# SciLifeLab/TIDDIT

Measured on AMD Instinct MI355X. Metric: cov bins/sec, 30x WGS synthetic (signals clustered/sec: see 'dbscan'), higher is better.
Workload: dtype int64; 1 GPU; BASELINE configs[1]: coverage histogram, 24 contigs x 125000000 bp (3.00 Gb), 30x 150-bp sorted stream, 500-bp bins, q>=20 filter; contigs split over the 1 rank(s); reads=600000000, bins=6000000

## Files before the change

tiddit_amd/csrc/tdt_coverage.hip:

```cpp
extern const char *const tdt_variant_coverage;
const char *const tdt_variant_coverage = ""
#ifdef COV_MIN_WAVES
    " COV_MIN_WAVES"
#endif
#ifdef COV_MIN_WAVES1
    " COV_MIN_WAVES1"
#endif
#ifdef COV_MIN_WAVES1_4
    " COV_MIN_WAVES1_4"
#endif
#ifdef COV_MIN_WAVES4
    " COV_MIN_WAVES4"
#endif
#ifdef COV_RPL
    " COV_RPL"
#endif
#ifdef COV_RPL1
    " COV_RPL1"
#endif
#ifdef COV_SPARES1
    " COV_SPARES1"
#endif
#ifdef COV_WIN
    " COV_WIN"
#endif
#ifdef COV_WIN1
    " COV_WIN1"
#endif
    ;

#include "tdt_common.h"

#include <algorithm>
#include <thread>

#define COV_THREADS 256
#ifndef COV_RPL
#define COV_RPL 8
#endif
#ifndef COV_RPL1
#define COV_RPL1 4
#endif
#define COV_READS_PER_BLOCK 16384
#ifndef COV_WIN
#define COV_WIN 2048
#endif
#define COV_LUT_LDS_MAX 1024
#define COV_PUSH_CHUNK (4u << 20)
#define COV_STATUS_BYTES (128 + COV_KEPT_SLOTS * 128)
#define COV_KEPT_SLOTS 512

struct CovItem {
    const int32_t *start;
    const int32_t *end;
    const uint8_t *mapq;
    const uint16_t *flag;
    const unsigned long long *packed;
    unsigned long long n;
    unsigned long long *acc;
    const unsigned long long *lut_end;
    int nbins;
    int aligned;
    unsigned first_block;
    unsigned binned;
};

struct CovParams {
    CovItem it;
    const CovItem *items;
    int n_items;
    int bin_size;
    unsigned magic;
    int shift;
    int min_q;
    int margin;
    unsigned xmax, m15;
    int k15;
    const unsigned long long *lut_main;
    unsigned long long one;
    int *status;
    unsigned long long *kept;
};

__device__ __forceinline__ int cov_div(int x, unsigned magic, int shift) {
    return shift < 0 ? x : (int)(__umulhi((unsigned)x, magic) >> shift);
}

#define DPP_WAVE_SHL1 0x130
#define DPP_WAVE_SHR1 0x138

template <int CTRL>
__device__ __forceinline__ unsigned long long dpp_u64(unsigned long long v) {
    const unsigned lo = __builtin_amdgcn_update_dpp(0u, (unsigned)v, CTRL, 0xf, 0xf, true);
    const unsigned hi = __builtin_amdgcn_update_dpp(0u, (unsigned)(v >> 32), CTRL, 0xf, 0xf, true);
    return ((unsigned long long)hi << 32) | lo;
}

#define COV_DPP_SHR1 "row_shr:1 row_mask:0xf bank_mask:0xf bound_ctrl:0"
#define COV_DPP_SHR2 "row_shr:2 row_mask:0xf bank_mask:0xf bound_ctrl:0"
#define COV_DPP_SHR4 "row_shr:4 row_mask:0xf bank_mask:0xf bound_ctrl:0"
#define COV_DPP_SHR8 "row_shr:8 row_mask:0xf bank_mask:0xf bound_ctrl:0"
#define COV_DPP_BC15 "row_bcast:15 row_mask:0xa bank_mask:0xf"
#define COV_DPP_BC31 "row_bcast:31 row_mask:0xc bank_mask:0xf"
#define COV_SCAN_ALL(STEP) \
    "s_nop 1\n\t" STEP(COV_DPP_SHR1) STEP(COV_DPP_SHR2) STEP(COV_DPP_SHR4) STEP(COV_DPP_SHR8) STEP(COV_DPP_BC15) STEP(COV_DPP_BC31) "s_nop 1"
#define COV_SCAN_STEP(CTRL)                                                                     \
    "v_add_co_u32_dpp %0, vcc, %0, %0 " CTRL "\n\t"                                             \
    "v_addc_co_u32_dpp %1, vcc, %1, %1, vcc " CTRL "\n\t"                                       \
    "v_add_co_u32_dpp %2, vcc, %2, %2 " CTRL "\n\t"                                             \
    "v_addc_co_u32_dpp %3, vcc, %3, %3, vcc " CTRL "\n\t"                                       \
    "v_add_co_u32_dpp %4, vcc, %4, %4 " CTRL "\n\t"                                             \
    "v_addc_co_u32_dpp %5, vcc, %5, %5, vcc " CTRL "\n\t"

__device__ __forceinline__ void wave_scan3_u64(unsigned long long &a0, unsigned long long &a1, unsigned long long &a2) {
    unsigned l0 = (unsigned)a0, h0 = (unsigned)(a0 >> 32), l1 = (unsigned)a1, h1 = (unsigned)(a1 >> 32),
             l2 = (unsigned)a2, h2 = (unsigned)(a2 >> 32);
    asm volatile(COV_SCAN_ALL(COV_SCAN_STEP) : "+v"(l0), "+v"(h0), "+v"(l1), "+v"(h1), "+v"(l2), "+v"(h2)::"vcc", "memory");
    a0 = ((unsigned long long)h0 << 32) | l0;
    a1 = ((unsigned long long)h1 << 32) | l1;
    a2 = ((unsigned long long)h2 << 32) | l2;
}

__device__ __forceinline__ unsigned long long cov_mask_lt(unsigned a, unsigned lim_uniform) {
    unsigned long long m;
    asm("v_cmp_gt_u32_e64 %0, %1, %2" : "=s"(m) : "s"(lim_uniform), "v"(a));
    return m;
}
__device__ __forceinline__ unsigned long long cov_mask_eq0(unsigned a) {
    unsigned long long m;
    asm("v_cmp_eq_u32_e64 %0, 0, %1" : "=s"(m) : "v"(a));
    return m;
}
__device__ __forceinline__ unsigned long long cov_mask_ne0(unsigned a) {
    unsigned long long m;
    asm("v_cmp_ne_u32_e64 %0, 0, %1" : "=s"(m) : "v"(a));
    return m;
}
__device__ __forceinline__ unsigned cov_select(unsigned long long m, unsigned if_set, unsigned if_clear) {
    unsigned r;
    asm("v_cndmask_b32_e64 %0, %1, %2, %3" : "=v"(r) : "v"(if_clear), "v"(if_set), "s"(m));
    return r;
}

#define COV_SCAN2_STEP(CTRL)                                                                    \
    "v_add_co_u32_dpp %0, vcc, %0, %0 " CTRL "\n\t"                                             \
    "v_addc_co_u32_dpp %1, vcc, %1, %1, vcc " CTRL "\n\t"                                       \
    "v_add_co_u32_dpp %2, vcc, %2, %2 " CTRL "\n\t"                                             \
    "v_addc_co_u32_dpp %3, vcc, %3, %3, vcc " CTRL "\n\t"

__device__ __forceinline__ void wave_scan2_u64(unsigned long long &a0, unsigned long long &a1) {
    unsigned l0 = (unsigned)a0, h0 = (unsigned)(a0 >> 32), l1 = (unsigned)a1, h1 = (unsigned)(a1 >> 32);
    asm volatile(COV_SCAN_ALL(COV_SCAN2_STEP) : "+v"(l0), "+v"(h0), "+v"(l1), "+v"(h1)::"vcc", "memory");
    a0 = ((unsigned long long)h0 << 32) | l0;
    a1 = ((unsigned long long)h1 << 32) | l1;
}

#define COV_SCAN4I_STEP(CTRL)                                                                   \
    "v_add_u32_dpp %0, %0, %0 " CTRL "\n\t"                                                     \
    "v_add_u32_dpp %1, %1, %1 " CTRL "\n\t"                                                     \
    "v_add_u32_dpp %2, %2, %2 " CTRL "\n\t"                                                     \
    "v_add_u32_dpp %3, %3, %3 " CTRL "\n\t"

__device__ __forceinline__ void wave_scan4_i32(int &p0, int &p1, int &p2, int &p3) {
    asm volatile(COV_SCAN_ALL(COV_SCAN4I_STEP) : "+v"(p0), "+v"(p1), "+v"(p2), "+v"(p3)::"memory");
}

__device__ __forceinline__ ulonglong2 cov_lds_read128(unsigned addr) {
#if defined(__HIP_DEVICE_COMPILE__)
    typedef unsigned long long cov_v2u64 __attribute__((ext_vector_type(2)));
    const cov_v2u64 v = *reinterpret_cast<const cov_v2u64 __attribute__((address_space(3))) *>(addr);
    return make_ulonglong2(v.x, v.y);
#else
    (void)addr;
    return make_ulonglong2(0, 0);
#endif
}

__device__ __forceinline__ unsigned long long cov_lds_read64(unsigned addr) {
#if defined(__HIP_DEVICE_COMPILE__)
    return *reinterpret_cast<const unsigned long long __attribute__((address_space(3))) *>(addr);
#else
    return addr;
#endif
}
__device__ __forceinline__ void cov_lds_add64(unsigned addr, unsigned long long v) {
#if defined(__HIP_DEVICE_COMPILE__)
    __hip_atomic_fetch_add(reinterpret_cast<unsigned long long __attribute__((address_space(3))) *>(addr), v, __ATOMIC_RELAXED, __HIP_MEMORY_SCOPE_WORKGROUP);
#else
    (void)addr; (void)v;
#endif
}
__device__ __forceinline__ unsigned cov_add_bit(unsigned r, unsigned long long mask) {
    unsigned out;
    unsigned long long cout;
    asm("v_addc_co_u32_e64 %0, %1, %2, 0, %3" : "=v"(out), "=s"(cout) : "v"(r), "s"(mask));
    return out;
}

__device__ __noinline__ void cov_global_add(unsigned long long *acc, int bin, unsigned long long v) {
    atomicAdd(&acc[bin], v);
}

template <int RPL>
struct CovTile {
    int s[RPL], e[RPL];
    unsigned mq[RPL / 4];
    unsigned fl[RPL / 2];
};

template <int RPL>
__device__ __forceinline__ CovTile<RPL> cov_load(const CovItem &P, unsigned long long idx, unsigned long long r1) {
    CovTile<RPL> t;
    if (P.aligned && idx + RPL <= r1) {
#pragma unroll
        for (int k = 0; k < RPL / 4; k++) {
            const int4 s4 = *reinterpret_cast<const int4 *>(P.start + idx + 4 * k);
            const int4 e4 = *reinterpret_cast<const int4 *>(P.end + idx + 4 * k);
            t.s[4 * k] = s4.x; t.s[4 * k + 1] = s4.y; t.s[4 * k + 2] = s4.z; t.s[4 * k + 3] = s4.w;
            t.e[4 * k] = e4.x; t.e[4 * k + 1] = e4.y; t.e[4 * k + 2] = e4.z; t.e[4 * k + 3] = e4.w;
        }
        if (RPL == 8) {
            const uint2 m2 = *reinterpret_cast<const uint2 *>(P.mapq + idx);
            const uint4 f4 = *reinterpret_cast<const uint4 *>(P.flag + idx);
            t.mq[0] = m2.x; t.mq[RPL / 4 - 1] = m2.y;
            t.fl[0] = f4.x; t.fl[1] = f4.y; t.fl[RPL / 2 - 2] = f4.z; t.fl[RPL / 2 - 1] = f4.w;
        } else {
            t.mq[0] = *reinterpret_cast<const unsigned *>(P.mapq + idx);
            const uint2 f2 = *reinterpret_cast<const uint2 *>(P.flag + idx);
            t.fl[0] = f2.x; t.fl[1] = f2.y;
        }
    } else {
#pragma unroll
        for (int k = 0; k < RPL / 4; k++) t.mq[k] = 0;
#pragma unroll
        for (int k = 0; k < RPL / 2; k++) t.fl[k] = 0;
#pragma unroll
        for (int j = 0; j < RPL; j++) {
            const bool ok = idx + j < r1;
            t.s[j] = ok ? P.start[idx + j] : 0;
            t.e[j] = ok ? P.end[idx + j] : 1;
            t.mq[j / 4] |= (ok ? (unsigned)P.mapq[idx + j] : 0u) << (8 * (j & 3));
            t.fl[j / 2] |= (ok ? (unsigned)P.flag[idx + j] : 0x4u) << (16 * (j & 1));
        }
    }
    return t;
}

template <int RPL>
struct CovTileP {
    unsigned long long w[RPL];
};

template <int RPL>
__device__ __forceinline__ CovTileP<RPL> cov_load_packed(const CovItem &P, unsigned long long idx, unsigned long long r1) {
    CovTileP<RPL> t;
    if (P.aligned && idx + RPL <= r1) {
#pragma unroll
        for (int k = 0; k < RPL / 2; k++) {
            const ulonglong2 v = *reinterpret_cast<const ulonglong2 *>(P.packed + idx + 2 * k);
            t.w[2 * k] = v.x;
            t.w[2 * k + 1] = v.y;
        }
    } else {
#pragma unroll
        for (int j = 0; j < RPL; j++) t.w[j] = idx + j < r1 ? P.packed[idx + j] : (1ull << 62);
    }
    return t;
}

__global__ void cov_pack(const int32_t *__restrict__ start, const int32_t *__restrict__ end, const uint8_t *__restrict__ mapq,
                         const uint16_t *__restrict__ flag, unsigned long long n, unsigned long long *__restrict__ out) {
    unsigned long long i = (unsigned long long)blockIdx.x * blockDim.x + threadIdx.x;
    const unsigned long long stride = (unsigned long long)gridDim.x * blockDim.x;
    for (; i < n; i += stride) out[i] = cov_pack_record(start[i], end[i], mapq[i], flag[i]);
}

__global__ void cov_pack_binned(const int32_t *__restrict__ start, const int32_t *__restrict__ end, const uint8_t *__restrict__ mapq,
                                const uint16_t *__restrict__ flag, unsigned long long n, int nbins, unsigned z, unsigned magic, int shift, int mode1,
                                unsigned long long *__restrict__ out) {
    unsigned long long i = (unsigned long long)blockIdx.x * blockDim.x + threadIdx.x;
    const unsigned long long stride = (unsigned long long)gridDim.x * blockDim.x;
    for (; i < n; i += stride) out[i] = cov_bin_record(start[i], end[i], mapq[i], flag[i], nbins, z, magic, shift, mode1 != 0);
}

#define COV_DBIT 48
#define COV_LOWMASK ((1ull << COV_DBIT) - 1ull)
#ifndef COV_WIN1
#define COV_WIN1 2048
#endif
#define COV_DQMAX 256
#ifndef COV_SPARES1
#define COV_SPARES1 64
#endif

#ifndef COV_MIN_WAVES
#define COV_MIN_WAVES 4
#endif
#ifndef COV_MIN_WAVES4
#define COV_MIN_WAVES4 3
#endif
#ifndef COV_MIN_WAVES1
#define COV_MIN_WAVES1 6
#endif
#ifndef COV_MIN_WAVES1_4
#define COV_MIN_WAVES1_4 4
#endif
template <bool LDS_LUT, int MODE, bool Z1, int RPL, int REC>
__global__ __launch_bounds__(COV_THREADS, MODE == 1 ? (REC ? COV_MIN_WAVES1 : COV_MIN_WAVES1_4) : (REC ? COV_MIN_WAVES : COV_MIN_WAVES4)) void cov_accumulate(CovParams P) {
    constexpr bool PACKED = REC != 0;
    extern __shared__ __attribute__((aligned(16))) unsigned long long smem[];
    constexpr int WIN = MODE == 1 ? COV_WIN1 : COV_WIN;
    constexpr int TILE = COV_THREADS * RPL;
    int *s_wsum = reinterpret_cast<int *>(smem);
    int *s_tbin = s_wsum + 4;
    int *s_rtot = reinterpret_cast<int *>(smem + 12);
    unsigned long long *win = smem + 12 + (MODE == 1 ? 16 : 0);
    unsigned long long *lutS = win + WIN + (MODE == 1 ? COV_SPARES1 : 2);

    const int tid = threadIdx.x;
    const int lane = tid & 63;
    CovItem I = P.it;
    unsigned blk = blockIdx.x;
    if (P.n_items > 0) {
        int lo = 0, hi = P.n_items;
        while (hi - lo > 1) {
            const int mid = (lo + hi) >> 1;
            if (P.items[mid].first_block <= blk) lo = mid;
            else hi = mid;
        }
        I = P.items[lo];
        blk -= I.first_block;
    }
    const unsigned long long r0 = (unsigned long long)blk * COV_READS_PER_BLOCK;
    const unsigned long long r1 = min(I.n, r0 + COV_READS_PER_BLOCK);
    const unsigned z = (unsigned)P.bin_size;
    const int last_bin = I.nbins - 1;
    auto div = [&](int x) { return Z1 ? x : (int)(__umulhi((unsigned)x, P.magic) >> P.shift); };

    auto load_tile = [&](unsigned long long idx) {
        if constexpr (PACKED) return cov_load_packed<RPL>(I, idx, r1);
        else return cov_load<RPL>(I, idx, r1);
    };
    auto cur = load_tile(r0 + (unsigned long long)tid * RPL);

    for (int i = tid; i < WIN + 2; i += COV_THREADS) win[i] = 0;
    if (LDS_LUT) {
        for (unsigned i = tid; i <= z; i += COV_THREADS) {
            const unsigned long long v = P.lut_main[i];
            lutS[i] = v;
            lutS[i + z + 1] = I.lut_end[i];
            if (MODE == 0 && !Z1) {
                unsigned long long *pr = lutS + 2 * (z + 1);
                pr[2 * i] = v;
                pr[2 * i + 1] = 0;
                pr[2 * (z + 1) + 2 * i] = 0;
                pr[2 * (z + 1) + 2 * i + 1] = v;
            }
            if (MODE == 1) {
                unsigned long long *tabA = lutS + 2 * (z + 1), *tabB = tabA + (z + 1), *tabL = tabB + (z + 1);
                tabA[i] = v & 0xffffffffull;
                tabB[i] = v << 32;
                tabL[i] = v - (1ull << COV_DBIT);
                if (i == 0) tabL[z + 1] = 0;
            }
        }
    }
    auto bin_of_read = [&](unsigned long long idx) {
        if constexpr (REC == 2) return (int)((unsigned)I.packed[idx] >> 2);
        int s = PACKED ? (int)(unsigned)I.packed[idx] : I.start[idx];
        s = s < 0 ? 0 : s;
        const int b = div(s);
        return b < I.nbins ? b : I.nbins - 1;
    };
    if (tid < COV_READS_PER_BLOCK / TILE) {
        const unsigned long long tl = min(r0 + (unsigned long long)(tid + 1) * TILE, r1) - 1;
        s_tbin[tid] = bin_of_read(tl);
    }
    int base = bin_of_read(r0);
    __syncthreads();
    auto lut = [&](unsigned i) -> unsigned long long {
        if (LDS_LUT) return lutS[i];
        return i <= z ? P.lut_main[i] : I.lut_end[i - z - 1];
    };

    auto contribute = [&](int bin, unsigned long long v) {
        const unsigned off = (unsigned)(bin - base);
        if (off < (unsigned)WIN) atomicAdd(&win[off], v);
        else if ((unsigned)bin <= (unsigned)last_bin) cov_global_add(I.acc, bin, v);
    };

    auto slow_read = [&](int s, int e) {
        const int fb = div(s);
        const int eb = div(e - 1);
        if (fb == eb) {
            contribute(fb, lut((unsigned)(e - s)));
        } else {
            contribute(fb, lut((unsigned)(fb + 1) * z - (unsigned)s));
            const unsigned bl = (unsigned)(e - 1) - (unsigned)eb * z;
            contribute(eb, lut(eb < last_bin ? bl : bl + z + 1));
            for (int b = fb + 1; b < eb; b++) contribute(b, P.one);
        }
    };

    auto spill = [&]() {
        __syncthreads();
        if constexpr (MODE == 1) {
            constexpr int PER = WIN / COV_THREADS;
            static_assert(PER == 8 && COV_THREADS == 256, "the packed resolve is written for eight rows of 256 words");
            unsigned long long w[PER];
#pragma unroll
            for (int k = 0; k < PER; k++) w[k] = win[k * COV_THREADS + tid];
            int pk[PER / 2];
#pragma unroll
            for (int j = 0; j < PER / 2; j++)
                pk[j] = (int)((long long)w[2 * j] >> COV_DBIT) + (int)((unsigned)((long long)w[2 * j + 1] >> COV_DBIT) << 16);
            wave_scan4_i32(pk[0], pk[1], pk[2], pk[3]);
            int incl[PER];
#pragma unroll
            for (int j = 0; j < PER / 2; j++) {
                incl[2 * j] = (int)(short)(pk[j] & 0xffff);
                incl[2 * j + 1] = (pk[j] - incl[2 * j]) >> 16;
            }
            const int wv = tid >> 6;
            if (lane == 63) {
#pragma unroll
                for (int k = 0; k < PER; k++) s_rtot[k * 4 + wv] = incl[k];
            }
            __syncthreads();
            int tot = lane < 4 * PER ? s_rtot[lane] : 0, z1 = 0, z2 = 0, z3 = 0;
            const int own = tot;
            wave_scan4_i32(tot, z1, z2, z3);
            const int excl = tot - own;
            const unsigned sh = (unsigned)__builtin_ctzll(P.one);
#pragma unroll
            for (int k = 0; k < PER; k++) {
                const int run = incl[k] + __builtin_amdgcn_readlane(excl, k * 4 + wv);
                const unsigned long long v = (w[k] & COV_LOWMASK) + ((unsigned long long)(long long)run << sh);
                const int i = k * COV_THREADS + tid;
                if (w[k]) win[i] = 0;
                if (v) {
                    if (base + i <= last_bin) atomicAdd(&I.acc[base + i], v);
                }
            }
            __syncthreads();
            return;
        }
        for (int i = tid; i < WIN; i += COV_THREADS) {
            const unsigned long long v = win[i];
            if (v) {
                if (base + i <= last_bin) atomicAdd(&I.acc[base + i], v);
                win[i] = 0;
            }
        }
    };

    unsigned nkept = 0;
    unsigned nkept_s = 0;
    bool bad = false;

    for (unsigned long long t0 = r0; t0 < r1; t0 += TILE) {
        auto nxt = cur;
        if (t0 + TILE < r1) nxt = load_tile(t0 + TILE + (unsigned long long)tid * RPL);

        if (t0 != r0) {
            const int step = (int)((t0 - r0) / TILE);
            if (s_tbin[step] + P.margin >= base + WIN) {
                const int nb = s_tbin[step - 1];
                if (nb != base) {
                    spill();
                    __syncthreads();
                    base = nb;
                }
            }
        }

        if constexpr (REC == 2) {
            static_assert(LDS_LUT && !Z1, "binned records exist for 2 <= bin_size < 1024");
            const unsigned K4 = (unsigned)cur.w[0] & ~3u;
            const int K = (int)(K4 >> 2);
            const unsigned ko = (unsigned)(K - base);
            const unsigned minq24 = (unsigned)P.min_q << 24, qlim = (64u - (unsigned)P.min_q) << 24;
            unsigned long long slow_any = 0;
            unsigned long long a0 = 0, a1 = 0, a2 = 0;
            if constexpr (MODE == 0) {
                const bool safe = ko < (unsigned)(WIN - 3);
                const unsigned kw = safe ? ko : 0u;
                const unsigned tA = (unsigned)(size_t)(lutS + 2 * (z + 1)), zb4 = (z + 1u) << 2;
                const unsigned notsafe = safe ? 0u : 8u;
#pragma unroll
                for (int j = 0; j < RPL; j++) {
                    const unsigned lo = (unsigned)cur.w[j], hi = (unsigned)(cur.w[j] >> 32);
                    const unsigned d = lo - K4;
                    const unsigned long long m_cand = cov_mask_lt(hi - minq24, qlim);
                    const unsigned long long m_fast = m_cand & cov_mask_eq0((d & ~5u) | notsafe);
                    nkept_s += (unsigned)__builtin_popcountll(m_fast);
                    slow_any |= m_cand & ~m_fast;
                    const unsigned tab = __umul24(d & 4u, zb4) + tA;
                    const unsigned xa = cov_select(m_fast, (hi & 0x3ff0u) + tab, tA);
                    const ulonglong2 X = cov_lds_read128(xa);
                    const unsigned long long m_multi = m_fast & cov_mask_ne0(d & 1u);
                    const unsigned ya = cov_select(m_multi, (((hi >> 14) & 0x3ffu) << 4) + tab, tA);
                    const ulonglong2 Y = cov_lds_read128(ya);
                    a0 += X.x;
                    a1 += X.y + Y.x;
                    a2 += Y.y;
                }
                if (slow_any) {
                    const unsigned long long idx = t0 + (unsigned long long)tid * RPL;
#pragma unroll
                    for (int j = 0; j < RPL; j++) {
                        unsigned lo = (unsigned)cur.w[j], hi = (unsigned)(cur.w[j] >> 32);
                        asm volatile("" : "+v"(lo), "+v"(hi));
                        const unsigned d = lo - K4;
                        if ((hi - minq24 < qlim) && !(safe & ((d & ~5u) == 0u))) {
                            if ((lo & 3u) == COV_BN_INVALID || idx + j >= r1) bad = true;
                            else { nkept++; slow_read(I.start[idx + j], I.end[idx + j]); }
                        }
                    }
                }
                if (a2) atomicAdd(&win[kw + 2], a2);
                wave_scan2_u64(a0, a1);
                const int Kprev = (int)__builtin_amdgcn_update_dpp((unsigned)~K, (unsigned)K, DPP_WAVE_SHR1, 0xf, 0xf, false);
                const int Knext = (int)__builtin_amdgcn_update_dpp((unsigned)~K, (unsigned)K, DPP_WAVE_SHL1, 0xf, 0xf, false);
                const unsigned long long q0 = dpp_u64<DPP_WAVE_SHR1>(a0), q1 = dpp_u64<DPP_WAVE_SHR1>(a1);
                if (safe && Knext != K) {
                    if (a0) atomicAdd(&win[kw], a0);
                    if (a1) atomicAdd(&win[kw + 1], a1);
                }
                if (safe && Kprev != K && lane != 0) {
                    if (q0) atomicAdd(&win[kw], 0ull - q0);
                    if (q1) atomicAdd(&win[kw + 1], 0ull - q1);
// ... 136 lines not shown
                    }
            }
            wave_scan3_u64(a0, a1, a2);
            const int Kprev = (int)__builtin_amdgcn_update_dpp((unsigned)~K, (unsigned)K, DPP_WAVE_SHR1, 0xf, 0xf, false);
            const int Knext = (int)__builtin_amdgcn_update_dpp((unsigned)~K, (unsigned)K, DPP_WAVE_SHL1, 0xf, 0xf, false);
            const unsigned long long q0 = dpp_u64<DPP_WAVE_SHR1>(a0), q1 = dpp_u64<DPP_WAVE_SHR1>(a1), q2 = dpp_u64<DPP_WAVE_SHR1>(a2);
            if (safe && Knext != K) {
                if (a0) atomicAdd(&win[kw], a0);
                if (a1) atomicAdd(&win[kw + 1], a1);
                if (a2) atomicAdd(&win[kw + 2], a2);
            }
            if (safe && Kprev != K && lane != 0) {
                if (q0) atomicAdd(&win[kw], 0ull - q0);
                if (q1) atomicAdd(&win[kw + 1], 0ull - q1);
                if (q2) atomicAdd(&win[kw + 2], 0ull - q2);
            }
        } else if (MODE == 0) {
#pragma unroll
            for (int j = 0; j < RPL; j++) {
                const int s = sv[j], e = ev[j];
                bool keep = !(fl[j] & FMASK) && (int)mq[j] >= P.min_q;
                const bool invalid = keep && (s < 0 || e <= s);
                const unsigned rs = (unsigned)s - Kz;
                const unsigned re = (unsigned)(e - 1) - Kz;
                const unsigned r = (rs >= z) ? 1u : 0u;
                const unsigned q = (re >= z ? 1u : 0u) + (re >= 2u * z ? 1u : 0u);
                const bool over = keep && !invalid && (K + (int)q > last_bin) && re < 3u * z;
                bad = bad || invalid || over;
                keep = keep && !invalid && !over;
                nkept += keep ? 1u : 0u;
                const bool fast = rs < 2u * z && re < 3u * z && q - r <= 1u;
                const bool ok = keep && fast;
                slowmask |= (keep && !fast) ? (1u << j) : 0u;
                const bool multi = q != r;
                const unsigned bf = multi ? (r + 1u) * z - rs : (unsigned)(e - s);
                const unsigned bl = re - q * z + ((K + (int)q == last_bin) ? z + 1u : 0u);
                const unsigned long long vF = lut(ok ? bf : 0u);
                const unsigned long long vL = lut((ok && multi) ? bl : 0u);
                const bool r0_ = r == 0;
                a0 += r0_ ? vF : 0ull;
                a1 += r0_ ? vL : vF;
                a2 += r0_ ? 0ull : vL;
            }
            if (slowmask) {
#pragma unroll
                for (int j = 0; j < RPL; j++)
                    if (slowmask & (1u << j)) {
                        if (div(ev[j] - 1) > last_bin) { bad = true; nkept--; }
                        else slow_read(sv[j], ev[j]);
                    }
            }
            wave_scan3_u64(a0, a1, a2);
            const int Kprev = (int)__builtin_amdgcn_update_dpp((unsigned)~K, (unsigned)K, DPP_WAVE_SHR1, 0xf, 0xf, false);
            const int Knext = (int)__builtin_amdgcn_update_dpp((unsigned)~K, (unsigned)K, DPP_WAVE_SHL1, 0xf, 0xf, false);
            const unsigned long long q0 = dpp_u64<DPP_WAVE_SHR1>(a0), q1 = dpp_u64<DPP_WAVE_SHR1>(a1), q2 = dpp_u64<DPP_WAVE_SHR1>(a2);
            if (Knext != K) {
                if (a0) contribute(K, a0);
                if (a1) contribute(K + 1, a1);
                if (a2) contribute(K + 2, a2);
            }
            if (Kprev != K && lane != 0) {
                if (q0) contribute(K, 0ull - q0);
                if (q1) contribute(K + 1, 0ull - q1);
                if (q2) contribute(K + 2, 0ull - q2);
            }
        } else {
            const unsigned long long *tabA = lutS + 2 * (z + 1), *tabL = tabA + 2 * (z + 1);
            const unsigned ko = (unsigned)(K - base);
            const bool safe = ko < (unsigned)(WIN - COV_DQMAX - 2) && K + COV_DQMAX + 2 <= last_bin;
            const unsigned kw = safe ? ko : 0u;
            unsigned d1 = 0, d2 = 0;
            unsigned long long vL[RPL];
            unsigned woff[RPL];
#pragma unroll
            for (int j = 0; j < RPL; j++) {
                const unsigned rs = (unsigned)sv[j] - Kz;
                const unsigned re1 = (unsigned)ev[j] - Kz;
                const unsigned len = re1 - rs;
                bool cand;
                if constexpr (PACKED) cand = (unsigned)(cur.w[j] >> 32) - ((unsigned)P.min_q << 24) < ((64u - (unsigned)P.min_q) << 24);
                else cand = ((fl[j] & FMASK) == 0) & ((int)mq[j] >= P.min_q);
                const bool fast = cand & safe & (rs < 2u * z) & (len - 1u < P.xmax) & (re1 <= P.xmax);
                nkept += fast ? 1u : 0u;
                slowmask |= (cand & !fast) ? (1u << j) : 0u;
                const bool r1_ = rs >= z;
                const unsigned dq = (__umul24(re1, P.m15) - P.m15) >> P.k15;
                const bool multi = fast & (dq != (r1_ ? 1u : 0u));
                const unsigned bf = min(len, (r1_ ? 2u * z : z) - rs);
                const unsigned long long vv = tabA[(fast ? bf : 0u) + (r1_ ? z + 1u : 0u)];
                a0 += (unsigned)vv;
                a1 += (unsigned)(vv >> 32);
                d1 += (multi & !r1_) ? 1u : 0u;
                d2 += (multi & r1_) ? 1u : 0u;
                const unsigned bl1 = re1 - __umul24(dq, z);
                vL[j] = tabL[multi ? bl1 - 1u : z + 1u];
                woff[j] = multi ? kw + dq : (unsigned)WIN;
            }
#pragma unroll
            for (int j = 0; j < RPL; j++) atomicAdd(&win[woff[j]], vL[j]);
            atomicAdd(&win[kw], a0);
            atomicAdd(&win[kw + 1], a1 + ((unsigned long long)d1 << COV_DBIT));
            atomicAdd(&win[kw + 2], (unsigned long long)d2 << COV_DBIT);
            if (slowmask) {
#pragma unroll
                for (int j = 0; j < RPL; j++)
                    if (slowmask & (1u << j)) {
                        const int s = sv[j], e = true_end(j);
                        if (s < 0 || e <= s || div(e - 1) > last_bin) bad = true;
                        else { nkept++; slow_read(s, e); }
                    }
            }
        }
        cur = nxt;
    }

    for (int d = 32; d > 0; d >>= 1) nkept += __shfl_down(nkept, d);
    nkept += nkept_s;
    if (lane == 0 && nkept)
        atomicAdd(P.kept + (size_t)((blockIdx.x * (COV_THREADS / 64) + (tid >> 6)) % COV_KEPT_SLOTS) * 16, (unsigned long long)nkept);
    if (bad) atomicOr(P.status, 1);

    spill();
}

__global__ void cov_finalize(const long long *__restrict__ acc, double *__restrict__ out, long long n, double inv_scale,
                             int *status) {
    long long i = (long long)blockIdx.x * blockDim.x + threadIdx.x;
    const long long stride = (long long)gridDim.x * blockDim.x;
    bool inexact = false;
    for (; i < n; i += stride) {
        const long long a = acc[i];
        if (a >= (1ll << 53) || a < 0) inexact = true;
        out[i] = (double)a * inv_scale;
    }
    if (inexact) atomicOr(status, 2);
}

struct tdt_cov {
    tdt_ctx *ctx = nullptr;
    int n_contigs = 0;
    int bin_size = 0;
    int S = 0;
    bool small_bins = false;
    unsigned xmax = 0, m15 = 0;
    int k15 = 0;
    unsigned magic = 0;
    int shift = 0;
    std::vector<int64_t> len, nbins, off;
    std::vector<int> end_bin_size;
    int64_t total_bins = 0;
    unsigned long long *d_acc = nullptr;
    unsigned long long *d_lut_main = nullptr;
    unsigned long long *d_lut_end = nullptr;
    int *d_status = nullptr;
    unsigned long long *d_kept = nullptr;
    int *d_nbins = nullptr;
    void *d_stage[2] = {nullptr, nullptr};
    void *h_stage[2] = {nullptr, nullptr};
    hipEvent_t slot_ev[2] = {nullptr, nullptr};
    int slot_used[2] = {0, 0};
    int next_slot = 0;
};

static bool build_lut(std::vector<unsigned long long> &lut, int bin_size, int den, int S) {
    const double scale = ldexp(1.0, S);
    for (int b = 0; b <= bin_size; b++) {
        volatile float q = (float)b / (float)den;
        double f = (double)q * scale;
        unsigned long long fx = (unsigned long long)f;
        if ((double)fx != f) return false;
        lut[b] = fx;
    }
    return true;
}

extern "C" int tdt_cov_create(tdt_ctx *ctx, const int64_t *contig_len, int n_contigs, int bin_size, tdt_cov **out) {
    if (!ctx || !contig_len || !out || n_contigs <= 0) {
        tdt_set_error("tdt_cov_create: bad argument");
        return TDT_E_ARG;
    }
    *out = nullptr;
    if (bin_size <= 0 || bin_size > (1 << 24)) {
        tdt_set_error("tdt_cov_create: bin_size %d outside [1, 2^24] (reference: float32 bases are exact only there)",
                      bin_size);
        return TDT_E_ARG;
    }
    TDT_HIP(hipSetDevice(ctx->device));
    tdt_cov *c = new tdt_cov();
    c->ctx = ctx;
    c->n_contigs = n_contigs;
    c->bin_size = bin_size;
    const int L = tdt_ceil_log2_u64((uint64_t)bin_size);
    c->S = 23 + L + 1;
    {
        const char *env = getenv("TIDDIT_COV_MODE");
        const bool can = bin_size >= 2 && c->S <= 31;
        c->small_bins = can;
        if (env && env[0] == '0') c->small_bins = false;
        if (bin_size >= 2 && bin_size + 1 <= COV_LUT_LDS_MAX) {
            c->k15 = 15 + L;
            c->m15 = (unsigned)(((1ull << c->k15) + (unsigned)bin_size - 1) / (unsigned)bin_size);
            const unsigned lim = (unsigned)COV_DQMAX * (unsigned)bin_size;
            c->xmax = lim < 32768u ? lim : 32768u;
            for (unsigned x = 0; x < 32768u; x++)
                if (((x * c->m15) >> c->k15) != x / (unsigned)bin_size) {
                    tdt_set_error("internal: 24-bit division self-check failed for d=%d x=%u", bin_size, x);
                    delete c;
                    return TDT_E_ARG;
                }
        }
    }
    if (L == 0) {
        c->shift = -1;
        c->magic = 0;
    } else {
        const unsigned __int128 num = (unsigned __int128)1 << (31 + L);
        const unsigned __int128 m = (num + (unsigned)bin_size - 1) / (unsigned)bin_size;
        c->magic = (unsigned)m;
        c->shift = L - 1;
        const int probes[] = {0, 1, bin_size - 1, bin_size, bin_size + 1, 2 * bin_size - 1, 2 * bin_size, 1000003,
                              0x3fffffff, 0x7ffffffe, 0x7fffffff};
        for (int x : probes) {
            if (x < 0) continue;
            const int q = (int)(((unsigned long long)(unsigned)x * c->magic) >> 32 >> c->shift);
            if (q != x / bin_size) {
                tdt_set_error("internal: magic division self-check failed for d=%d x=%d", bin_size, x);
                delete c;
                return TDT_E_ARG;
            }
        }
    }
    c->len.assign(contig_len, contig_len + n_contigs);
    c->nbins.resize(n_contigs);
    c->off.resize(n_contigs);
    c->end_bin_size.resize(n_contigs);
    int64_t total = 0;
    for (int i = 0; i < n_contigs; i++) {
        const int64_t LN = contig_len[i];
        if (LN < 0 || LN > 0x7fffffffll) {
            tdt_set_error("tdt_cov_create: contig %d length %lld outside [0, 2^31)", i, (long long)LN);
            delete c;
            return TDT_E_ARG;
        }
        const int64_t bins = (LN + bin_size - 1) / bin_size;
        c->nbins[i] = bins;
        c->end_bin_size[i] = (int)(LN - (bins - 1) * bin_size);
        c->off[i] = total;
        total += bins;
        total = (total + 1) & ~1ll;
    }
    c->total_bins = total;
    const size_t lut_n = (size_t)bin_size + 1;
    std::vector<unsigned long long> lut(lut_n), lute((size_t)n_contigs * lut_n);
    if (!build_lut(lut, bin_size, bin_size, c->S)) {
        tdt_set_error("internal: fixed-point scale 2^-%d cannot represent float32(b)/float32(%d)", c->S, bin_size);
        delete c;
        return TDT_E_ARG;
    }
    for (int i = 0; i < n_contigs; i++) {
        std::vector<unsigned long long> t(lut_n);
        const int ebs = c->end_bin_size[i] > 0 ? c->end_bin_size[i] : bin_size;
        const double scale = ldexp(1.0, c->S);
        for (size_t b = 0; b < lut_n; b++) {
            volatile float q = (float)b / (float)ebs;
            double f = (double)q * scale;
            unsigned long long fx = (f < 9007199254740992.0) ? (unsigned long long)f : 0ull;
            t[b] = (f < 9007199254740992.0 && (double)fx == f) ? fx : (1ull << 53);
        }
        memcpy(&lute[(size_t)i * lut_n], t.data(), lut_n * sizeof(unsigned long long));
    }
    hipError_t e;
    auto fail = [&](const char *what) {
        tdt_set_error("tdt_cov_create: %s failed: %s", what, hipGetErrorString(e));
        tdt_cov_destroy(c);
        return TDT_E_HIP;
    };
    if ((e = tdt_dev_malloc((void **)&c->d_acc, (size_t)(total > 0 ? total : 1) * 8)) != hipSuccess) return fail("hipMalloc(acc)");
    if ((e = tdt_dev_malloc((void **)&c->d_lut_main, lut_n * 8)) != hipSuccess) return fail("hipMalloc(lut)");
    if ((e = tdt_dev_malloc((void **)&c->d_lut_end, (size_t)n_contigs * lut_n * 8)) != hipSuccess) return fail("hipMalloc(lut_end)");
    if ((e = tdt_dev_malloc((void **)&c->d_status, COV_STATUS_BYTES)) != hipSuccess) return fail("hipMalloc(status)");
    {
        std::vector<int> nb32(c->nbins.begin(), c->nbins.end());
        if ((e = tdt_dev_malloc((void **)&c->d_nbins, (size_t)n_contigs * 4)) != hipSuccess) return fail("hipMalloc(nbins)");
        if ((e = hipMemcpy(c->d_nbins, nb32.data(), (size_t)n_contigs * 4, hipMemcpyHostToDevice)) != hipSuccess) return fail("hipMemcpy(nbins)");
    }
    c->d_kept = (unsigned long long *)((char *)c->d_status + 128);
    if ((e = hipMemcpy(c->d_lut_main, lut.data(), lut_n * 8, hipMemcpyHostToDevice)) != hipSuccess) return fail("hipMemcpy(lut)");
    if ((e = hipMemcpy(c->d_lut_end, lute.data(), (size_t)n_contigs * lut_n * 8, hipMemcpyHostToDevice)) != hipSuccess)
        return fail("hipMemcpy(lut_end)");
    if ((e = hipMemset(c->d_acc, 0, (size_t)(total > 0 ? total : 1) * 8)) != hipSuccess) return fail("hipMemset(acc)");
    if ((e = hipMemset(c->d_status, 0, COV_STATUS_BYTES)) != hipSuccess) return fail("hipMemset(status)");
    for (int i = 0; i < 2; i++)
        if ((e = hipEventCreateWithFlags(&c->slot_ev[i], hipEventDisableTiming)) != hipSuccess) return fail("hipEventCreate");
    *out = c;
    return TDT_OK;
}

extern "C" void tdt_cov_destroy(tdt_cov *c) {
    if (!c) return;
    (void)hipSetDevice(c->ctx->device);
    (void)hipStreamSynchronize(c->ctx->stream);
    if (c->d_acc) (void)hipFree(c->d_acc);
    if (c->d_lut_main) (void)hipFree(c->d_lut_main);
    if (c->d_lut_end) (void)hipFree(c->d_lut_end);
    if (c->d_status) (void)hipFree(c->d_status);
    if (c->d_nbins) (void)hipFree(c->d_nbins);
    for (int i = 0; i < 2; i++) {
        if (c->d_stage[i]) (void)hipFree(c->d_stage[i]);
        if (c->h_stage[i]) (void)hipHostFree(c->h_stage[i]);
        if (c->slot_ev[i]) (void)hipEventDestroy(c->slot_ev[i]);
    }
    delete c;
}

extern "C" int tdt_cov_nbins(tdt_cov *c, int tid, int64_t *nbins, int *end_bin_size) {
    if (!c || tid < 0 || tid >= c->n_contigs) {
        tdt_set_error("tdt_cov_nbins: bad contig id");
        return TDT_E_ARG;
    }
    if (nbins) *nbins = c->nbins[tid];
    if (end_bin_size) *end_bin_size = c->end_bin_size[tid];
    return TDT_OK;
}

extern "C" int tdt_cov_scale_bits(tdt_cov *c) { return c ? c->S : TDT_E_ARG; }

extern "C" int tdt_cov_reset(tdt_cov *c) {
    if (!c) return TDT_E_ARG;
    TDT_HIP(hipSetDevice(c->ctx->device));
    TDT_HIP(hipMemsetAsync(c->d_acc, 0, (size_t)(c->total_bins > 0 ? c->total_bins : 1) * 8, c->ctx->stream));
    TDT_HIP(hipMemsetAsync(c->d_status, 0, COV_STATUS_BYTES, c->ctx->stream));
    return TDT_OK;
}

static CovItem cov_item(tdt_cov *c, int tid, const int32_t *d_start, const int32_t *d_end, const uint8_t *d_mapq,
                        const uint16_t *d_flag, size_t n) {
    CovItem it;
    it.start = d_start;
    it.end = d_end;
    it.mapq = d_mapq;
    it.flag = d_flag;
    it.packed = nullptr;
    it.n = n;
    it.acc = c->d_acc + c->off[tid];
    it.lut_end = c->d_lut_end + (size_t)tid * ((size_t)c->bin_size + 1);
    it.nbins = (int)c->nbins[tid];
    it.aligned = (((uintptr_t)d_start | (uintptr_t)d_end) & 15) == 0 && ((uintptr_t)d_mapq & (COV_RPL - 1)) == 0 &&
                 ((uintptr_t)d_flag & (2 * COV_RPL - 1)) == 0;
    it.first_block = 0;
    it.binned = 0;
    return it;
}

static CovItem cov_item_packed(tdt_cov *c, int tid, const unsigned long long *d_packed, const int32_t *d_end, size_t n) {
    CovItem it = cov_item(c, tid, nullptr, d_end, nullptr, nullptr, n);
    it.packed = d_packed;
    it.aligned = ((uintptr_t)d_packed & 15) == 0;
    return it;
}

static int cov_launch_items(tdt_cov *c, const CovItem &single, const CovItem *d_items, int n_items, unsigned grid, int min_q) {
    CovParams P;
    P.it = single;
    P.items = d_items;
    P.n_items = n_items;
    P.bin_size = c->bin_size;
    P.magic = c->magic;
    P.shift = c->shift;
    P.min_q = min_q;
    P.lut_main = c->d_lut_main;
    P.one = 1ull << c->S;
    P.status = c->d_status;
    P.kept = c->d_kept;
    const bool small = c->small_bins;
    P.margin = small ? COV_DQMAX + 8 : 640 / c->bin_size + 4;
    P.xmax = c->xmax;
    P.m15 = c->m15;
    P.k15 = c->k15;
    const bool lds_lut = c->bin_size + 1 <= COV_LUT_LDS_MAX;
    const size_t lds = 96 + (small ? 128 : 0) + ((size_t)(small ? COV_WIN1 + COV_SPARES1 : COV_WIN + 2)) * 8 + (lds_lut ? 2 * ((size_t)c->bin_size + 1) * 8 : 0) +
                       (small ? (3 * ((size_t)c->bin_size + 1) + 1) * 8 : 0) + ((!small && lds_lut && c->shift >= 0) ? 4 * ((size_t)c->bin_size + 1) * 8 : 0);
    const bool packed = single.packed != nullptr;
    const bool binned = packed && single.binned;
    if (binned && small)
        hipLaunchKernelGGL((cov_accumulate<true, 1, false, COV_RPL1, 2>), dim3(grid), dim3(COV_THREADS), lds, c->ctx->stream, P);
    else if (binned)
        hipLaunchKernelGGL((cov_accumulate<true, 0, false, COV_RPL, 2>), dim3(grid), dim3(COV_THREADS), lds, c->ctx->stream, P);
    else if (small && packed)
        hipLaunchKernelGGL((cov_accumulate<true, 1, false, COV_RPL1, 1>), dim3(grid), dim3(COV_THREADS), lds, c->ctx->stream, P);
    else if (small)
        hipLaunchKernelGGL((cov_accumulate<true, 1, false, COV_RPL1, 0>), dim3(grid), dim3(COV_THREADS), lds, c->ctx->stream, P);
    else if (lds_lut && c->shift >= 0 && packed)
        hipLaunchKernelGGL((cov_accumulate<true, 0, false, COV_RPL, 1>), dim3(grid), dim3(COV_THREADS), lds, c->ctx->stream, P);
    else if (lds_lut && c->shift >= 0)
        hipLaunchKernelGGL((cov_accumulate<true, 0, false, COV_RPL, 0>), dim3(grid), dim3(COV_THREADS), lds, c->ctx->stream, P);
    else if (lds_lut && packed)
        hipLaunchKernelGGL((cov_accumulate<true, 0, true, COV_RPL, 1>), dim3(grid), dim3(COV_THREADS), lds, c->ctx->stream, P);
    else if (lds_lut)
        hipLaunchKernelGGL((cov_accumulate<true, 0, true, COV_RPL, 0>), dim3(grid), dim3(COV_THREADS), lds, c->ctx->stream, P);
    else if (packed)
        hipLaunchKernelGGL((cov_accumulate<false, 0, false, COV_RPL, 1>), dim3(grid), dim3(COV_THREADS), lds, c->ctx->stream, P);
    else
        hipLaunchKernelGGL((cov_accumulate<false, 0, false, COV_RPL, 0>), dim3(grid), dim3(COV_THREADS), lds, c->ctx->stream, P);
    TDT_CHECK_LAUNCH();
    return TDT_OK;
}

static int cov_launch(tdt_cov *c, int tid, const int32_t *d_start, const int32_t *d_end, const uint8_t *d_mapq,
                      const uint16_t *d_flag, size_t n, int min_q) {
    if (n == 0 || c->nbins[tid] == 0) return TDT_OK;
    const unsigned grid = (unsigned)((n + COV_READS_PER_BLOCK - 1) / COV_READS_PER_BLOCK);
    return cov_launch_items(c, cov_item(c, tid, d_start, d_end, d_mapq, d_flag, n), nullptr, 0, grid, min_q);
}

extern "C" int tdt_cov_push_device_multi(tdt_cov *c, int n_items, const int *tids, const int32_t *const *d_start,
                                         const int32_t *const *d_end, const uint8_t *const *d_mapq,
                                         const uint16_t *const *d_flag, const size_t *n, int min_q) {
    if (!c || n_items < 0 || (n_items && (!tids || !d_start || !d_end || !d_mapq || !d_flag || !n))) {
        tdt_set_error("tdt_cov_push_device_multi: bad argument");
        return TDT_E_ARG;
    }
    TDT_HIP(hipSetDevice(c->ctx->device));
    std::vector<CovItem> items;
    unsigned long long blocks = 0;
    for (int i = 0; i < n_items; i++) {
        if (tids[i] < 0 || tids[i] >= c->n_contigs || (n[i] && (!d_start[i] || !d_end[i] || !d_mapq[i] || !d_flag[i]))) {
            tdt_set_error("tdt_cov_push_device_multi: bad item %d", i);
            return TDT_E_ARG;
        }
        if (n[i] == 0 || c->nbins[tids[i]] == 0) continue;
        CovItem it = cov_item(c, tids[i], d_start[i], d_end[i], d_mapq[i], d_flag[i], n[i]);
        it.first_block = (unsigned)blocks;
        blocks += (n[i] + COV_READS_PER_BLOCK - 1) / COV_READS_PER_BLOCK;
        items.push_back(it);
    }
    if (items.empty()) return TDT_OK;
    if (blocks >= 0x7fffffffull) {
        tdt_set_error("tdt_cov_push_device_multi: too many reads for one launch");
        return TDT_E_ARG;
    }
    void *d_items = nullptr;
    int rc = tdt_scratch(c->ctx, 7, items.size() * sizeof(CovItem), &d_items);
    if (rc) return rc;
    TDT_HIP(hipMemcpyAsync(d_items, items.data(), items.size() * sizeof(CovItem), hipMemcpyHostToDevice, c->ctx->stream));
    return cov_launch_items(c, items[0], (const CovItem *)d_items, (int)items.size(), (unsigned)blocks, min_q);
}

extern "C" int tdt_cov_pack_device(tdt_ctx *ctx, const int32_t *d_start, const int32_t *d_end, const uint8_t *d_mapq, const uint16_t *d_flag,
                                   size_t n, uint64_t *d_packed) {
    if (!ctx || (n && (!d_start || !d_end || !d_mapq || !d_flag || !d_packed))) {
        tdt_set_error("tdt_cov_pack_device: bad argument");
        return TDT_E_ARG;
    }
    if (!n) return TDT_OK;
    TDT_HIP(hipSetDevice(ctx->device));
    size_t blocks = (n + 255) / 256;
    if (blocks > 65536) blocks = 65536;
    hipLaunchKernelGGL(cov_pack, dim3((unsigned)blocks), dim3(256), 0, ctx->stream, d_start, d_end, d_mapq, d_flag, (unsigned long long)n,
                       (unsigned long long *)d_packed);
    TDT_CHECK_LAUNCH();
    return TDT_OK;
}

extern "C" int tdt_cov_push_packed_device_multi(tdt_cov *c, int n_items, const int *tids, const uint64_t *const *d_packed,
                                                const int32_t *const *d_end, const size_t *n, int min_q) {
    if (!c || n_items < 0 || (n_items && (!tids || !d_packed || !n))) {
        tdt_set_error("tdt_cov_push_packed_device_multi: bad argument");
        return TDT_E_ARG;
    }
    if (min_q > 63) {
        tdt_set_error("tdt_cov_push_packed_device_multi: packed records keep min(mapq, 63); min_q %d needs the unpacked entry point", min_q);
        return TDT_E_UNSUPPORTED;
    }
    if (min_q < 0) min_q = 0;
    TDT_HIP(hipSetDevice(c->ctx->device));
    std::vector<CovItem> items;
    unsigned long long blocks = 0;
    for (int i = 0; i < n_items; i++) {
        if (tids[i] < 0 || tids[i] >= c->n_contigs || (n[i] && !d_packed[i])) {
            tdt_set_error("tdt_cov_push_packed_device_multi: bad item %d", i);
            return TDT_E_ARG;
        }
        if (n[i] == 0 || c->nbins[tids[i]] == 0) continue;
        CovItem it = cov_item_packed(c, tids[i], (const unsigned long long *)d_packed[i], d_end ? d_end[i] : nullptr, n[i]);
        it.first_block = (unsigned)blocks;
        blocks += (n[i] + COV_READS_PER_BLOCK - 1) / COV_READS_PER_BLOCK;
        items.push_back(it);
    }
    if (items.empty()) return TDT_OK;
    if (blocks >= 0x7fffffffull) {
        tdt_set_error("tdt_cov_push_packed_device_multi: too many reads for one launch");
        return TDT_E_ARG;
    }
    void *d_items = nullptr;
    int rc = tdt_scratch(c->ctx, 7, items.size() * sizeof(CovItem), &d_items);
    if (rc) return rc;
    TDT_HIP(hipMemcpyAsync(d_items, items.data(), items.size() * sizeof(CovItem), hipMemcpyHostToDevice, c->ctx->stream));
    return cov_launch_items(c, items[0], (const CovItem *)d_items, (int)items.size(), (unsigned)blocks, min_q);
}

int tdt_cov_bin_spec(tdt_cov *c, CovBinSpec *out) {
    *out = CovBinSpec();
    if (!c) return TDT_E_ARG;
    if (c->bin_size < 2 || c->bin_size + 1 > COV_LUT_LDS_MAX) return TDT_OK;
    out->z = (unsigned)c->bin_size;
    out->magic = c->magic;
    out->shift = c->shift;
    out->mode1 = c->small_bins ? 1 : 0;
    out->d_nbins = c->d_nbins;
    out->n_contigs = c->n_contigs;
    return TDT_OK;
}

extern "C" int tdt_cov_pack_binned_device(tdt_cov *c, int tid, const int32_t *d_start, const int32_t *d_end, const uint8_t *d_mapq,
                                          const uint16_t *d_flag, size_t n, uint64_t *d_binned) {
    if (!c || tid < 0 || tid >= c->n_contigs || (n && (!d_start || !d_end || !d_mapq || !d_flag || !d_binned))) {
        tdt_set_error("tdt_cov_pack_binned_device: bad argument");
        return TDT_E_ARG;
    }
    CovBinSpec sp;
    tdt_cov_bin_spec(c, &sp);
    if (!sp.z) {
        tdt_set_error("tdt_cov_pack_binned_device: binned records exist for 2 <= bin_size < 1024 (this histogram: %d)", c->bin_size);
        return TDT_E_UNSUPPORTED;
    }
    if (!n) return TDT_OK;
    TDT_HIP(hipSetDevice(c->ctx->device));
    size_t blocks = (n + 255) / 256;
    if (blocks > 65536) blocks = 65536;
    hipLaunchKernelGGL(cov_pack_binned, dim3((unsigned)blocks), dim3(256), 0, c->ctx->stream, d_start, d_end, d_mapq, d_flag, (unsigned long long)n,
                       (int)c->nbins[tid], sp.z, sp.magic, sp.shift, sp.mode1, (unsigned long long *)d_binned);
    TDT_CHECK_LAUNCH();
    return TDT_OK;
}
// ... 214 lines not shown
```

Before: 6.526 billion bins/s.

## Prebuild LDS lookup-table image on host and bulk-copy it with 128-bit loads

Instead of each block computing the derived LUT tables (pairs, split halves, minus-delta) element by element with scalar stores in the prologue, the host prebuilds a flat image in the exact LDS layout. Each block then copies it with 16-byte global loads, issued early so they overlap the first read-tile loads, the window clear and the tile-bin lookups. The per-contig end table is spliced into its slot. The aim is to shorten the per-block setup before the main loop. It adds an extra device buffer and tricky slot-boundary handling, and it limits small-bin mode to bin sizes up to 128.

Result: no change. 6.486 billion bins/s, median of 2 (-0.6%).

```diff
diff --git a/tiddit_amd/csrc/tdt_cov_lut_image.h b/tiddit_amd/csrc/tdt_cov_lut_image.h
--- /dev/null
+++ b/tiddit_amd/csrc/tdt_cov_lut_image.h
@@ -0,0 +1,30 @@
+#pragma once
+#include <cstddef>
+#include <vector>
+
+#define COV_DBIT 48
+
+enum { COV_IMG_PLAIN = 0, COV_IMG_PAIRS = 1, COV_IMG_SMALL = 2 };
+
+static inline size_t cov_lut_image_words(int bin_size, int flavour) {
+    const size_t n = (size_t)bin_size + 1;
+    const size_t w = flavour == COV_IMG_PAIRS ? 6 * n : flavour == COV_IMG_SMALL ? 5 * n + 1 : 2 * n;
+    return (w + 1) & ~(size_t)1;
+}
+
+static inline void cov_lut_image_build(const unsigned long long *lut_main, int bin_size, int flavour, std::vector<unsigned long long> &img) {
+    const size_t n = (size_t)bin_size + 1;
+    img.assign(cov_lut_image_words(bin_size, flavour), 0ull);
+    for (size_t i = 0; i < n; i++) {
+        const unsigned long long v = lut_main[i];
+        img[i] = v;
+        if (flavour == COV_IMG_PAIRS) {
+            img[2 * n + 2 * i] = v;
+            img[4 * n + 2 * i + 1] = v;
+        } else if (flavour == COV_IMG_SMALL) {
+            img[2 * n + i] = v & 0xffffffffull;
+            img[3 * n + i] = v << 32;
+            img[4 * n + i] = v - (1ull << COV_DBIT);
+        }
+    }
+}
diff --git a/tiddit_amd/csrc/tdt_coverage.hip b/tiddit_amd/csrc/tdt_coverage.hip
--- a/tiddit_amd/csrc/tdt_coverage.hip
+++ b/tiddit_amd/csrc/tdt_coverage.hip
@@ -30,6 +30,7 @@
     ;
 
 #include "tdt_common.h"
+#include "tdt_cov_lut_image.h"
 
 #include <algorithm>
 #include <thread>
@@ -77,6 +78,8 @@
     unsigned xmax, m15;
     int k15;
     const unsigned long long *lut_main;
+    const unsigned long long *lut_img;
+    unsigned img_units;
     unsigned long long one;
     int *status;
     unsigned long long *kept;
@@ -165,9 +168,35 @@
     asm volatile(COV_SCAN_ALL(COV_SCAN4I_STEP) : "+v"(p0), "+v"(p1), "+v"(p2), "+v"(p3)::"memory");
 }
 
+typedef unsigned long long cov_v2u64 __attribute__((ext_vector_type(2)));
+
+template <typename T>
+__device__ __forceinline__ cov_v2u64 cov_gload128(const T *p) {
+#if defined(__HIP_DEVICE_COMPILE__)
+    return *reinterpret_cast<const cov_v2u64 __attribute__((address_space(1))) *>((uintptr_t)p);
+#else
+    return *reinterpret_cast<const cov_v2u64 *>(p);
+#endif
+}
+template <typename T>
+__device__ __forceinline__ unsigned long long cov_gload64(const T *p) {
+#if defined(__HIP_DEVICE_COMPILE__)
+    return *reinterpret_cast<const unsigned long long __attribute__((address_space(1))) *>((uintptr_t)p);
+#else
+    return *reinterpret_cast<const unsigned long long *>(p);
+#endif
+}
+template <typename T>
+__device__ __forceinline__ unsigned cov_gload32(const T *p) {
+#if defined(__HIP_DEVICE_COMPILE__)
+    return *reinterpret_cast<const unsigned __attribute__((address_space(1))) *>((uintptr_t)p);
+#else
+    return *reinterpret_cast<const unsigned *>(p);
+#endif
+}
+
 __device__ __forceinline__ ulonglong2 cov_lds_read128(unsigned addr) {
 #if defined(__HIP_DEVICE_COMPILE__)
-    typedef unsigned long long cov_v2u64 __attribute__((ext_vector_type(2)));
     const cov_v2u64 v = *reinterpret_cast<const cov_v2u64 __attribute__((address_space(3))) *>(addr);
     return make_ulonglong2(v.x, v.y);
 #else
@@ -283,11 +312,11 @@
     for (; i < n; i += stride) out[i] = cov_bin_record(start[i], end[i], mapq[i], flag[i], nbins, z, magic, shift, mode1 != 0);
 }
 
-#define COV_DBIT 48
 #define COV_LOWMASK ((1ull << COV_DBIT) - 1ull)
 #ifndef COV_WIN1
 #define COV_WIN1 2048
 #endif
+#define COV_SMALL_ZMAX 128
 #define COV_DQMAX 256
 #ifndef COV_SPARES1
 #define COV_SPARES1 64
@@ -343,40 +372,71 @@
     };
     auto cur = load_tile(r0 + (unsigned long long)tid * RPL);
 
-    for (int i = tid; i < WIN + 2; i += COV_THREADS) win[i] = 0;
-    if (LDS_LUT) {
-        for (unsigned i = tid; i <= z; i += COV_THREADS) {
-            const unsigned long long v = P.lut_main[i];
-            lutS[i] = v;
-            lutS[i + z + 1] = I.lut_end[i];
-            if (MODE == 0 && !Z1) {
-                unsigned long long *pr = lutS + 2 * (z + 1);
-                pr[2 * i] = v;
-                pr[2 * i + 1] = 0;
-                pr[2 * (z + 1) + 2 * i] = 0;
-                pr[2 * (z + 1) + 2 * i + 1] = v;
-            }
-            if (MODE == 1) {
-                unsigned long long *tabA = lutS + 2 * (z + 1), *tabB = tabA + (z + 1), *tabL = tabB + (z + 1);
-                tabA[i] = v & 0xffffffffull;
-                tabB[i] = v << 32;
-                tabL[i] = v - (1ull << COV_DBIT);
-                if (i == 0) tabL[z + 1] = 0;
-            }
-        }
-    }
-    auto bin_of_read = [&](unsigned long long idx) {
-        if constexpr (REC == 2) return (int)((unsigned)I.packed[idx] >> 2);
-        int s = PACKED ? (int)(unsigned)I.packed[idx] : I.start[idx];
+    constexpr int IMG_RU = MODE == 1 ? 2 : (Z1 ? 1 : 6);
+    constexpr int END_N = (MODE == 1 || Z1) ? 1 : COV_LUT_LDS_MAX / COV_THREADS;
+    constexpr int IMG_ROUNDS = (MODE == 0 && !Z1) ? 2 : 1;
+    static_assert(!LDS_LUT || (size_t)IMG_ROUNDS * IMG_RU * COV_THREADS * 2 >= (MODE == 1 ? 5 * (COV_SMALL_ZMAX + 1) + 1 : Z1 ? 4 : 6 * COV_LUT_LDS_MAX),
+                  "the image rounds cover the largest image of the flavour");
+    static_assert(!LDS_LUT || END_N * COV_THREADS >= (MODE == 1 ? COV_SMALL_ZMAX + 1 : Z1 ? 2 : COV_LUT_LDS_MAX), "the end-table share covers bin_size + 1 entries");
+    const unsigned slot0 = z + 1u;
+    cov_v2u64 im[IMG_RU];
+    auto img_load = [&](unsigned u0) {
+#pragma unroll
+        for (int k = 0; k < IMG_RU; k++) {
+            const unsigned u = u0 + (unsigned)tid + (unsigned)k * COV_THREADS;
+            im[k] = cov_gload128(P.lut_img + 2u * min(u, P.img_units - 1u));
+        }
+    };
+    auto img_store = [&](unsigned u0) {
+#pragma unroll
+        for (int k = 0; k < IMG_RU; k++) {
+            const unsigned u = u0 + (unsigned)tid + (unsigned)k * COV_THREADS, w0 = 2u * u;
+            if (u < P.img_units && w0 + 1u - slot0 > z + 1u) *reinterpret_cast<cov_v2u64 *>(lutS + w0) = im[k];
+        }
+    };
+    unsigned long long le[END_N];
+    if constexpr (LDS_LUT) {
+        img_load(0);
+#pragma unroll
+        for (int k = 0; k < END_N; k++) le[k] = cov_gload64(I.lut_end + min((unsigned)tid + (unsigned)k * COV_THREADS, z));
+    }
+    auto first_word = [&](unsigned long long idx) { return PACKED ? cov_gload32(I.packed + idx) : cov_gload32(I.start + idx); };
+    auto bin_of_word = [&](unsigned w) {
+        if constexpr (REC == 2) return (int)(w >> 2);
+        int s = (int)w;
         s = s < 0 ? 0 : s;
         const int b = div(s);
         return b < I.nbins ? b : I.nbins - 1;
     };
-    if (tid < COV_READS_PER_BLOCK / TILE) {
-        const unsigned long long tl = min(r0 + (unsigned long long)(tid + 1) * TILE, r1) - 1;
-        s_tbin[tid] = bin_of_read(tl);
-    }
-    int base = bin_of_read(r0);
+    unsigned w_tile = 0;
+    if (tid < COV_READS_PER_BLOCK / TILE) w_tile = first_word(min(r0 + (unsigned long long)(tid + 1) * TILE, r1) - 1);
+    const unsigned w_base = first_word(r0);
+
+    static_assert((WIN + 2) % 2 == 0, "the window is cleared in 16-byte units");
+    for (int i = tid; i < (WIN + 2) / 2; i += COV_THREADS) *reinterpret_cast<cov_v2u64 *>(win + 2 * i) = cov_v2u64{0ull, 0ull};
+    asm volatile("" : "+v"(w_tile));
+
+    if constexpr (LDS_LUT) {
+        img_store(0);
+#pragma unroll
+        for (int k = 0; k < END_N; k++) {
+            const unsigned i = (unsigned)tid + (unsigned)k * COV_THREADS;
+            if (i <= z) lutS[slot0 + i] = le[k];
+        }
+        if constexpr (IMG_RU >= 2) {
+            static_assert(IMG_RU < 2 || COV_LUT_LDS_MAX <= 4 * COV_THREADS, "the unit around the slot's start is one of a thread's first two");
+            const unsigned us = z >> 1;
+            if ((slot0 & 1u) && (unsigned)tid == (us & (COV_THREADS - 1u))) lutS[z] = us >= COV_THREADS ? im[1].x : im[0].x;
+        }
+        if constexpr (IMG_ROUNDS == 2) {
+            if (P.img_units > (unsigned)(IMG_RU * COV_THREADS)) {
+                img_load(IMG_RU * COV_THREADS);
+                img_store(IMG_RU * COV_THREADS);
+            }
+        }
+    }
+    if (tid < COV_READS_PER_BLOCK / TILE) s_tbin[tid] = bin_of_word(w_tile);
+    int base = bin_of_word(w_base);
     __syncthreads();
     auto lut = [&](unsigned i) -> unsigned long long {
         if (LDS_LUT) return lutS[i];
@@ -819,6 +879,9 @@
     unsigned long long *d_acc = nullptr;
     unsigned long long *d_lut_main = nullptr;
     unsigned long long *d_lut_end = nullptr;
+    unsigned long long *d_lut_img = nullptr;
+    int img_flavour = COV_IMG_PLAIN;
+    size_t img_words = 0;
     int *d_status = nullptr;
     unsigned long long *d_kept = nullptr;
     int *d_nbins = nullptr;
@@ -861,7 +924,7 @@
     c->S = 23 + L + 1;
     {
         const char *env = getenv("TIDDIT_COV_MODE");
-        const bool can = bin_size >= 2 && c->S <= 31;
+        const bool can = bin_size >= 2 && c->S <= 31 && bin_size <= COV_SMALL_ZMAX;
         c->small_bins = can;
         if (env && env[0] == '0') c->small_bins = false;
         if (bin_size >= 2 && bin_size + 1 <= COV_LUT_LDS_MAX) {
@@ -952,6 +1015,14 @@
         if ((e = hipMemcpy(c->d_nbins, nb32.data(), (size_t)n_contigs * 4, hipMemcpyHostToDevice)) != hipSuccess) return fail("hipMemcpy(nbins)");
     }
     c->d_kept = (unsigned long long *)((char *)c->d_status + 128);
+    if (bin_size + 1 <= COV_LUT_LDS_MAX) {
+        c->img_flavour = c->small_bins ? COV_IMG_SMALL : (c->shift >= 0 ? COV_IMG_PAIRS : COV_IMG_PLAIN);
+        std::vector<unsigned long long> img;
+        cov_lut_image_build(lut.data(), bin_size, c->img_flavour, img);
+        c->img_words = img.size();
+        if ((e = tdt_dev_malloc((void **)&c->d_lut_img, img.size() * 8)) != hipSuccess) return fail("hipMalloc(lut_img)");
+        if ((e = hipMemcpy(c->d_lut_img, img.data(), img.size() * 8, hipMemcpyHostToDevice)) != hipSuccess) return fail("hipMemcpy(lut_img)");
+    }
     if ((e = hipMemcpy(c->d_lut_main, lut.data(), lut_n * 8, hipMemcpyHostToDevice)) != hipSuccess) return fail("hipMemcpy(lut)");
     if ((e = hipMemcpy(c->d_lut_end, lute.data(), (size_t)n_contigs * lut_n * 8, hipMemcpyHostToDevice)) != hipSuccess)
         return fail("hipMemcpy(lut_end)");
@@ -970,6 +1041,7 @@
     if (c->d_acc) (void)hipFree(c->d_acc);
     if (c->d_lut_main) (void)hipFree(c->d_lut_main);
     if (c->d_lut_end) (void)hipFree(c->d_lut_end);
+    if (c->d_lut_img) (void)hipFree(c->d_lut_img);
     if (c->d_status) (void)hipFree(c->d_status);
     if (c->d_nbins) (void)hipFree(c->d_nbins);
     for (int i = 0; i < 2; i++) {
@@ -1036,6 +1108,8 @@
     P.shift = c->shift;
     P.min_q = min_q;
     P.lut_main = c->d_lut_main;
+    P.lut_img = c->d_lut_img;
+    P.img_units = (unsigned)(c->img_words / 2);
     P.one = 1ull << c->S;
     P.status = c->d_status;
     P.kept = c->d_kept;
@@ -1045,8 +1119,7 @@
     P.m15 = c->m15;
     P.k15 = c->k15;
     const bool lds_lut = c->bin_size + 1 <= COV_LUT_LDS_MAX;
-    const size_t lds = 96 + (small ? 128 : 0) + ((size_t)(small ? COV_WIN1 + COV_SPARES1 : COV_WIN + 2)) * 8 + (lds_lut ? 2 * ((size_t)c->bin_size + 1) * 8 : 0) +
-                       (small ? (3 * ((size_t)c->bin_size + 1) + 1) * 8 : 0) + ((!small && lds_lut && c->shift >= 0) ? 4 * ((size_t)c->bin_size + 1) * 8 : 0);
+    const size_t lds = 96 + (small ? 128 : 0) + ((size_t)(small ? COV_WIN1 + COV_SPARES1 : COV_WIN + 2)) * 8 + c->img_words * 8;
     const bool packed = single.packed != nullptr;
     const bool binned = packed && single.binned;
     if (binned && small)
```
